# aik2mlj/polyffusion

Hardware: AMD Instinct MI355X
Metric: denoising steps/sec (8-bar prmat2c, batch 16) (higher is better)
Workload: dtype bf16x3; 1 GPU; sdf_chd8bar cond generation, batch 16 per GPU, 1000-step DDPM sampler loop body (BASELINE.json configs[1]); weights: deterministic synthetic, 41.08M params; global_batch=16, parallelism=batch-shard x1

## Files before the change

polyffusion_amd/csrc/conv_bf16x3.hip:

```cpp
#include <vector>

#include "conv_common.h"

namespace pf {

#ifdef PF_TRACE
__device__ unsigned long long g_trace[8192];
#define TR() do { if (trace_on && tslot < 2040) { g_trace[tbase + tslot++] = __builtin_amdgcn_s_memtime(); } } while (0)
#else
#define TR() do {} while (0)
#endif

typedef x3_t x3x4 __attribute__((ext_vector_type(4)));

template <int KS, int STRIDE, int TWIN, int BN>
constexpr int conv_bf3_row_pitch() {
  return (KS != 1 && STRIDE == 1 && BN >= 128) ? (TWIN * 40 + 127) / 128 * 128 : TWIN * 40;
}

#ifndef PF_KG2_RING
#define PF_KG2_RING 5
#endif
template <int KS, int BN, int KG>
constexpr bool conv_bf3_pingpong() { return KS == 3 && BN == 128 && KG == 2; }
// ... 132 lines not shown
    {
      f32x4 v = ra[i];
      if (poff[i] < 0) v = f32x4{0.f, 0.f, 0.f, 0.f};
      else if (PRO != 0) {
        if (PRO == 3) {
          v = (v - pmu[i]) * prs[i] * vsc + vsh;
        } else {
          v = v * vsc + vsh;
          if (PRO == 1) { v[0] = silu_f(v[0]); v[1] = silu_f(v[1]); v[2] = silu_f(v[2]); v[3] = silu_f(v[3]); }
        }
      }
      qh[i] = __builtin_convertvector(v, x3x4);
      const f32x4 hf = __builtin_convertvector(qh[i], f32x4);
      ql[i] = __builtin_convertvector(v - hf, x3x4);
    }
  };
  auto transformA = [&]() {
#pragma unroll
    for (int i = 0; i < NA; ++i) transformPiece(i);
  };
  auto writeA = [&](int buf) {
#pragma unroll
    for (int i = 0; i < NA; ++i) {
      const int pix = tid / KQ + i * PSTEP;
      if (pix < NPIX) {
        const int o = buf * ABUF + (pix / TWIN) * RP + (pix % TWIN) * PITCH + c4 * 4;
        *reinterpret_cast<x3x4*>(sAh + o) = qh[i];
        *reinterpret_cast<x3x4*>(sAl + o) = ql[i];
      }
    }
  };
  auto storeA = [&](int buf) { transformA(); writeA(buf); };
  auto loadW = [&](int chunk, int tap) {
    const size_t toff = ((size_t)tap * K8 + (size_t)(cbeg + chunk) * 4) * ((size_t)2 * p.Npad * 8);
#pragma unroll
    for (int j = 0; j < NW; ++j) {
      const int u = tid + j * NT;
      const int k8l = u / (2 * BN), plane = (u / BN) & 1, n = u % BN;
      rw[j] = *reinterpret_cast<const u32x4*>(static_cast<const x3_t*>(p.w) + ((size_t)(k8l * 2 + plane) * p.Npad + n0 + n) * 8 + toff);
    }
  };
  auto storeW = [&](int buf) {
    x3_t* dst = sW + buf * (TOTW * 8);
#pragma unroll
    for (int j = 0; j < NW; ++j) {
      *reinterpret_cast<u32x4*>(dst + (tid + j * NT) * 8) = rw[j];
    }
  };

  static_assert(NT % (2 * BN) == 0, "pieces of a thread must be whole k8 rows apart");
  const int wrow_b = 2 * p.Npad * 8 * 2;
  const __amdgpu_buffer_rsrc_t rsW = dma_resource(static_cast<const x3_t*>(p.w) + (size_t)n0 * 8);
  const int vw0 = (((tid / (2 * BN)) * 2 + ((tid / BN) & 1)) * p.Npad + tid % BN) * 16;
  auto gldsW = [&](int chunk, int tap, int buf) {
    const int toff = ((q * TAPS + tap) * K8 + (cbeg + chunk) * 4) * wrow_b;
#pragma unroll
    for (int j = 0; j < NW; ++j) {
      x3_t* l = sW + buf * (TOTW * 8) + (wave * 64 + j * NT) * 8;
      dma16(rsW, vw0, toff + j * (NT / (2 * BN)) * wrow_b, l);
    }
  };

  int hbase[FM];
#pragma unroll
  for (int fm = 0; fm < FM; ++fm) {
    const int pp = wm * WM + fm * 32 + (lane & 31);
    const int py = pp / TW, px = pp % TW;
    hbase[fm] = (py * STRIDE) * RP + (px * STRIDE) * PITCH + 8 * (lane >> 5);
  }
  const int wbase = ((lane >> 5) * 2 * BN + wn * WN + (lane & 31)) * 8;

  f32x16 acc[FM][FN];
#pragma unroll
  for (int fm = 0; fm < FM; ++fm)
#pragma unroll
    for (int fn = 0; fn < FN; ++fn)
#pragma unroll
      for (int r = 0; r < 16; ++r) acc[fm][fn][r] = 0.f;


  auto gnFused = [&]() {
    if constexpr (PRO == 1 || PRO == 2) {
      if (p.gn_s0) {
        gn_fused_prologue<KG * NT>(p, b, threadIdx.x, p.Hin * p.Win, reinterpret_cast<double*>(smem_all));
        const int cg = cbeg * BK;
        vsc = *reinterpret_cast<const f32x4*>(p.sc + (size_t)b * cin + cg + c4 * 4);
        vsh = *reinterpret_cast<const f32x4*>(p.sh + (size_t)b * cin + cg + c4 * 4);
        sc_ready = true;
      }
    }
  };
  if constexpr (KS == 1) {
    loadA(0); loadW(0, 0);
    gnFused();
    storeA(0); storeW(0);
    __syncthreads();
    for (int chunk = 0; chunk < nchunk; ++chunk) {
      const int nchunk1 = min(chunk + 1, nchunk - 1);
      loadW(nchunk1, 0);
      loadA(nchunk1);
      const int aoff = (chunk & 1) * ABUF;
      const x3_t* cW = sW + (chunk & 1) * (TOTW * 8) + wbase;
#pragma unroll
      for (int s = 0; s < BK / 16; ++s) {
        x3x8 ah[FM], al[FM], bh[FN], bl[FN];
#pragma unroll
        for (int fm = 0; fm < FM; ++fm) {
          ah[fm] = *reinterpret_cast<const x3x8*>(sAh + aoff + hbase[fm] + s * 16);
          al[fm] = *reinterpret_cast<const x3x8*>(sAl + aoff + hbase[fm] + s * 16);
        }
#pragma unroll
        for (int fn = 0; fn < FN; ++fn) {
          bh[fn] = *reinterpret_cast<const x3x8*>(cW + ((4 * s) * BN + fn * 32) * 8);
          bl[fn] = *reinterpret_cast<const x3x8*>(cW + ((4 * s + 1) * BN + fn * 32) * 8);
        }
#pragma unroll
        for (int fm = 0; fm < FM; ++fm)
#pragma unroll
          for (int fn = 0; fn < FN; ++fn) acc[fm][fn] = x3_mfma_32x32x16(al[fm], bh[fn], acc[fm][fn], 0, 0, 0);
#pragma unroll
        for (int fm = 0; fm < FM; ++fm)
#pragma unroll
          for (int fn = 0; fn < FN; ++fn) acc[fm][fn] = x3_mfma_32x32x16(ah[fm], bl[fn], acc[fm][fn], 0, 0, 0);
#pragma unroll
        for (int fm = 0; fm < FM; ++fm)
#pragma unroll
          for (int fn = 0; fn < FN; ++fn) acc[fm][fn] = x3_mfma_32x32x16(ah[fm], bh[fn], acc[fm][fn], 0, 0, 0);
      }
      storeW((chunk + 1) & 1);
      storeA((chunk + 1) & 1);
      __syncthreads();
    }
  } else {
    constexpr int NS = BK / 16;
    static_assert(NS == 2 && WRING >= 2 && WRING <= TAPS, "pipeline is written for two K steps per tap and a ring no deeper than a chunk's taps");
    constexpr bool DYN = TAPS % WRING != 0;
    constexpr int NAL = NA + (PRO != 0 ? 2 : 0);
    constexpr bool PP = conv_bf3_pingpong<KS, BN, KG>();
#pragma unroll
    for (int d = 0; d < (PP ? 2 : WRING); ++d) gldsW(0, d, d);
    TR();
    loadA(0);
    TR();
    gnFused();
    storeA(0);
    TR();
    asm volatile("s_waitcnt vmcnt(0) lgkmcnt(0)" ::: "memory");
    __builtin_amdgcn_s_barrier();
    x3x8 ah[FM], al[FM], bh[FN], bl[FN];
    unsigned abase[FM];
#pragma unroll
    for (int fm = 0; fm < FM; ++fm) abase[fm] = (unsigned)(size_t)(__attribute__((address_space(3))) x3_t*)(sAh + hbase[fm]);
    const unsigned wb = (unsigned)(size_t)(__attribute__((address_space(3))) x3_t*)(sW + wbase);
    constexpr int ALO = APLANE * 2;
    constexpr int WSLOT = TOTW * 16;
    static_assert(ALO + (2 * RP + 2 * PITCH) * 2 + 64 < 65536 && (DYN ? 1 : WRING) * WSLOT < 65536, "LDS immediates must fit 16 bits");
#define LD_AL1(I, AOFF, S) al[I] = lds_read128<ALO + ((AOFF) + (S) * 16) * 2>(abase[I])
#define LD_AH1(I, AOFF, S) ah[I] = lds_read128<((AOFF) + (S) * 16) * 2>(abase[I])
#define LD_BH1(I, SLOT, S) bh[I] = lds_read128<(DYN ? 0 : slot_##SLOT * WSLOT) + ((4 * (S)) * BN + (I) * 32) * 16>(DYN ? wb_##SLOT : wb)
#define LD_BL1(I, SLOT, S) bl[I] = lds_read128<(DYN ? 0 : slot_##SLOT * WSLOT) + ((4 * (S) + 1) * BN + (I) * 32) * 16>(DYN ? wb_##SLOT : wb)
#define LD_AL(AOFF, S) static_for<0, FM>([&](auto i) { LD_AL1(i.value, AOFF, S); })
#define LD_AH(AOFF, S) static_for<0, FM>([&](auto i) { LD_AH1(i.value, AOFF, S); })
#define LD_BH(SLOT, S) static_for<0, FN>([&](auto i) { LD_BH1(i.value, SLOT, S); })
#define LD_BL(SLOT, S) static_for<0, FN>([&](auto i) { LD_BL1(i.value, SLOT, S); })
#define SB() __builtin_amdgcn_sched_barrier(0)
#define FENCE() asm volatile("" ::: "memory")
    constexpr int G = FM * FN;
    auto GX = [&](auto&& f) {
      static_for<0, FM>([&](auto fm) { static_for<0, FN>([&](auto fn) {
        acc[fm.value][fn.value] = x3_mfma_32x32x16(al[fm.value], bh[fn.value], acc[fm.value][fn.value], 0, 0, 0);
// ... 593 lines not shown
```

polyffusion_amd/csrc/conv_common.h:

```cpp
#pragma once
#include <type_traits>

#include "pf_internal.h"

namespace pf {

typedef x3_t x3x8 __attribute__((ext_vector_type(8)));
typedef unsigned int u32x4 __attribute__((ext_vector_type(4)));

template <int OFF>
__device__ __forceinline__ x3x8 lds_read128(unsigned addr) {
  u32x4 v;
  constexpr int HI = OFF & ~0xFFFF, LO = OFF & 0xFFFF;
  if constexpr (HI != 0) addr += HI;
  asm volatile("ds_read_b128 %0, %1 offset:%2" : "=v"(v) : "v"(addr), "n"(LO));
  return __builtin_bit_cast(x3x8, v);
}
__device__ __forceinline__ __amdgpu_buffer_rsrc_t dma_resource(const void* base) {
  return __builtin_amdgcn_make_buffer_rsrc(const_cast<void*>(base), 0, 0x7fffffff, 0x00020000);
}
__device__ __forceinline__ void dma16(__amdgpu_buffer_rsrc_t rs, int voff, int soff, void* lds_wave_base) {
  __builtin_amdgcn_raw_ptr_buffer_load_lds(rs, (__attribute__((address_space(3))) void*)lds_wave_base, 16, voff, soff, 0, 0);
}

template <int N>
__device__ __forceinline__ void lgkm_wait() { asm volatile("s_waitcnt lgkmcnt(%0)" ::"n"(N)); }
template <int I, int N, class F>
__device__ __forceinline__ void static_for(F&& f) {
  if constexpr (I < N) { f(std::integral_constant<int, I>{}); static_for<I + 1, N>(f); }
}


struct FastDiv { unsigned mul, shr; };
static inline FastDiv make_fastdiv(int d) {
  if (d <= 1) return FastDiv{0u, 0u};
  unsigned l = 31u - (unsigned)__builtin_clz((unsigned)d);
  if (d & (d - 1)) ++l;
  const unsigned p = 31u + l;
  return FastDiv{(unsigned)(((1ull << p) + (unsigned)d - 1u) / (unsigned)d), p - 32u};
}
__device__ __forceinline__ int fdiv(int x, FastDiv f) { return f.mul ? (int)(__umulhi((unsigned)x, f.mul) >> f.shr) : x; }

struct ConvP {
  const float* x0; const float* x1; int c0, c1;
  int B, Hin, Win, Hout, Wout;
  const void* w; int N, Npad;
  const float* sc; const float* sh; const float* mean; const float* rstd;
  const float* bias; const float* sbias; int ld_sbias; const float* res; int ld_res;
  const long long* sb_rows; int sb_nrows;
  int geglu;
  float* out; int ld_out;
  float* stats;
  int tiles_x, tiles_y, nt;
  FastDiv d_tx, d_ty, d_nt, d_ks;
  int fold, fold_py, fold_px;
  const float* sx0; const float* sx1; int sc0, sc1;
  const void* sw; const float* bias2;
  void* out_planes;
  void* qkv;
  int pp;
  int ksplit; float* partial;
  const float* gn_s0; const float* gn_s1; int gn_t0, gn_t1;
  const float* gn_gamma; const float* gn_beta; float gn_eps; int gn_groups;
  int x1_bmod;
  unsigned* amax;
};

__device__ __forceinline__ void conv_shared_x1(ConvP& p, int b) {
  if (p.x1_bmod > 0) {
    const size_t d = (size_t)(b - b % p.x1_bmod);
    if (p.x1) p.x1 -= d * ((size_t)p.Hin * p.Win * p.c1);
    if (p.sx1) p.sx1 -= d * ((size_t)p.Hout * p.Wout * p.sc1);
    if (p.gn_s1) p.gn_s1 -= d * ((size_t)p.gn_t1 * p.c1 * 2);
  }
}

static inline void conv_fill_divs(ConvP& p) {
  p.d_tx = make_fastdiv(p.tiles_x); p.d_ty = make_fastdiv(p.tiles_y); p.d_nt = make_fastdiv(p.nt); p.d_ks = make_fastdiv(p.ksplit);
}

template <int NTHREADS>
__device__ __forceinline__ void gn_fused_prologue(const ConvP& p, int b, int tid_wg, int hw, double* scratch) {
  const int cin = p.c0 + p.c1, gs = cin / p.gn_groups;
  for (int c = tid_wg; c < cin; c += NTHREADS) {
    const float* s; int T, C, cl;
    if (c < p.c0) { s = p.gn_s0; T = p.gn_t0; C = p.c0; cl = c; } else { s = p.gn_s1; T = p.gn_t1; C = p.c1; cl = c - p.c0; }
    double a = 0.0, q = 0.0;
    for (int t0 = 0; t0 < T; t0 += 8) {
      float2 vv[8];
#pragma unroll
      for (int j = 0; j < 8; ++j)
        vv[j] = *reinterpret_cast<const float2*>(s + (((size_t)b * T + min(t0 + j, T - 1)) * C + cl) * 2);
#pragma unroll
      for (int j = 0; j < 8; ++j)
        if (t0 + j < T) { a += vv[j].x; q += vv[j].y; }
    }
    scratch[2 * c] = a; scratch[2 * c + 1] = q;
  }
  __syncthreads();
  float* scw = const_cast<float*>(p.sc) + (size_t)b * cin;
  float* shw = const_cast<float*>(p.sh) + (size_t)b * cin;
  for (int c = tid_wg; c < cin; c += NTHREADS) {
    const int g0 = (c / gs) * gs;
    double a = 0.0, q = 0.0;
    for (int j = 0; j < gs; ++j) { a += scratch[2 * (g0 + j)]; q += scratch[2 * (g0 + j) + 1]; }
    const double cnt = (double)gs * hw;
    const double mean = a / cnt;
    double var = q / cnt - mean * mean;
    if (var < 0.0) var = 0.0;
    const double rstd = 1.0 / sqrt(var + (double)p.gn_eps);
    const double ga = p.gn_gamma[c];
    scw[c] = (float)(rstd * ga);
    shw[c] = (float)((double)p.gn_beta[c] - mean * rstd * ga);
  }
  __threadfence_block();
  __syncthreads();
}

__device__ __forceinline__ void amax_acc(unsigned& m, float v) { m = max(m, __float_as_uint(v) & 0x7fffffffu); }
__device__ __forceinline__ void amax_acc4(unsigned& m, f32x4 v) { amax_acc(m, v[0]); amax_acc(m, v[1]); amax_acc(m, v[2]); amax_acc(m, v[3]); }
__device__ __forceinline__ void amax_flush(unsigned* slot, unsigned m) {
  if (!slot) return;
#pragma unroll
  for (int o = 32; o >= 1; o >>= 1) m = max(m, (unsigned)__shfl_xor((int)m, o));
  if ((threadIdx.x & 63) == 0 && m) atomicMax(slot, m);
}

__device__ __forceinline__ float silu_f(float v) { return v * __builtin_amdgcn_rcpf(1.0f + __expf(-v)); }
__device__ __forceinline__ float erf_as_f(float x) {
  const float ax = fabsf(x);
  const float t = __builtin_amdgcn_rcpf(fmaf(0.3275911f, ax, 1.0f));
  float pq = fmaf(1.061405429f, t, -1.453152027f);
  pq = fmaf(pq, t, 1.421413741f);
  pq = fmaf(pq, t, -0.284496736f);
  pq = fmaf(pq, t, 0.254829592f);
  const float y = 1.0f - pq * t * __expf(-ax * ax);
  return copysignf(y, x);
}
__device__ __forceinline__ float gelu_erf_f(float g) { return 0.5f * g * (1.0f + erf_as_f(g * 0.70710678118654752440f)); }

__device__ __forceinline__ void store_out(const ConvP& p, size_t idx, float v) { p.out[idx] = v; }
__device__ __forceinline__ const float* sbias_row(const ConvP& p, int b) {
  if (!p.sbias) return nullptr;
  long long r = b;
  if (p.sb_rows) { r = p.sb_rows[b]; r = r < 0 ? 0 : (r >= p.sb_nrows ? p.sb_nrows - 1 : r); }
  return p.sbias + (size_t)r * p.ld_sbias;
}
__device__ __forceinline__ size_t out_pixel(const ConvP& p, int b, int oy, int ox) {
  if (p.fold) return ((size_t)b * (2 * p.Hout) + 2 * oy + p.fold_py) * (size_t)(2 * p.Wout) + 2 * ox + p.fold_px;
  return ((size_t)b * p.Hout + oy) * p.Wout + ox;
}

__device__ __forceinline__ void quad_transpose_s1(f32x4& a, int lane) {
  const bool p1 = lane & 1;
  float s0 = p1 ? a[0] : a[1], s1 = p1 ? a[2] : a[3];
  float r0 = __builtin_bit_cast(float, __builtin_amdgcn_mov_dpp(__builtin_bit_cast(int, s0), 0xB1, 0xF, 0xF, true));
  float r1 = __builtin_bit_cast(float, __builtin_amdgcn_mov_dpp(__builtin_bit_cast(int, s1), 0xB1, 0xF, 0xF, true));
  if (p1) { a[0] = r0; a[2] = r1; } else { a[1] = r0; a[3] = r1; }
}
__device__ __forceinline__ void quad_transpose_s2(f32x4& a, int lane) {
  const bool p2 = lane & 2;
  float s0 = p2 ? a[0] : a[2], s1 = p2 ? a[1] : a[3];
  float r0 = __builtin_bit_cast(float, __builtin_amdgcn_mov_dpp(__builtin_bit_cast(int, s0), 0x4E, 0xF, 0xF, true));
  float r1 = __builtin_bit_cast(float, __builtin_amdgcn_mov_dpp(__builtin_bit_cast(int, s1), 0x4E, 0xF, 0xF, true));
  if (p2) { a[0] = r0; a[1] = r1; } else { a[2] = r0; a[3] = r1; }
}
__device__ __forceinline__ void quad_transpose(f32x4& a, int lane) { quad_transpose_s1(a, lane); quad_transpose_s2(a, lane); }
__device__ __forceinline__ float quad_sum(float v) {
  v += __builtin_bit_cast(float, __builtin_amdgcn_mov_dpp(__builtin_bit_cast(int, v), 0xB1, 0xF, 0xF, true));
  v += __builtin_bit_cast(float, __builtin_amdgcn_mov_dpp(__builtin_bit_cast(int, v), 0x4E, 0xF, 0xF, true));
  return v;
}

template <int TH, int TW, int BN, int FM, int FN, int NWM = 2>
__device__ __forceinline__ void conv_epilogue(const ConvP& p, f32x16 (&acc)[FM][FN], int b, int oy0, int ox0, int n0,
                                              int wm, int wn, int lane, int tid, float* red, bool active = true) {
  constexpr int WM = TH * TW / NWM, WN = BN / 2;
  unsigned am = 0;
  if (!active) {
    if (p.stats && !p.partial) { __syncthreads(); __syncthreads(); }
    return;
  }
  if (p.partial) {
#pragma unroll
    for (int fm = 0; fm < FM; ++fm)
#pragma unroll
      for (int r = 0; r < 16; ++r) {
        const int row = (r & 3) + 8 * (r >> 2) + 4 * (lane >> 5);
        const int pp = wm * WM + fm * 32 + row;
        const int oy = oy0 + pp / TW, ox = ox0 + pp % TW;
        if (oy >= p.Hout || ox >= p.Wout) continue;
        const size_t m = out_pixel(p, b, oy, ox);
#pragma unroll
        for (int fn = 0; fn < FN; ++fn) {
          const int n = n0 + wn * WN + fn * 32 + (lane & 31);
          if (n < p.N) p.partial[m * p.N + n] = acc[fm][fn][r];
        }
// ... 334 lines not shown
```

polyffusion_amd/csrc/conv_wino.hip:

```cpp
#include "conv_common.h"

namespace pf {

typedef x3_t x3x4 __attribute__((ext_vector_type(4)));

#ifdef PF_TRACE
__device__ unsigned long long g_wtrace[3 * 256];
#define WTR() do { if (trace_on && tslot < 255) { g_wtrace[tbase + tslot++] = __builtin_amdgcn_s_memtime(); } } while (0)
#define WTR_DECL() const bool trace_on = (threadIdx.x == 0) && (blockIdx.x == 0 || blockIdx.x == gridDim.x / 2 || blockIdx.x == gridDim.x - 1); \
                   const int tbase = blockIdx.x == 0 ? 0 : (blockIdx.x == gridDim.x - 1 ? 512 : 256); int tslot = 0; (void)tbase
#else
#define WTR() do {} while (0)
#define WTR_DECL() do {} while (0)
#endif

constexpr int WPP = 36, WRP = 18 * WPP + 8, WHALO = 18 * WRP;
constexpr int WINO_LDS = 4 * 2 * 4 * 16 * 64 * 4;

__device__ __forceinline__ void lds_barrier() {
  asm volatile("s_waitcnt lgkmcnt(0)" ::: "memory");
  __builtin_amdgcn_s_barrier();
  asm volatile("" ::: "memory");
}

template <class T>
__device__ __forceinline__ const T* uniform_ptr(const T* q) {
  const unsigned long long v = reinterpret_cast<unsigned long long>(q);
  const unsigned lo = __builtin_amdgcn_readfirstlane((unsigned)v), hi = __builtin_amdgcn_readfirstlane((unsigned)(v >> 32));
  return reinterpret_cast<const T*>(((unsigned long long)hi << 32) | lo);
}

__device__ __forceinline__ __amdgpu_buffer_rsrc_t rsrc_or_empty(const void* q) {
  return __builtin_amdgcn_make_buffer_rsrc(const_cast<void*>(q), 0, q ? 0x7fffffff : 0, 0x00020000);
}
__device__ __forceinline__ const float* sbias_row_scalar(const ConvP& p, int b) {
  if (!p.sbias) return nullptr;
  long long r = b;
  if (p.sb_rows) {
    typedef const long long __attribute__((address_space(4))) * cptr;
    r = *((cptr)(unsigned long long)(p.sb_rows + b));
    r = r < 0 ? 0 : (r >= p.sb_nrows ? p.sb_nrows - 1 : r);
  }
  return p.sbias + (size_t)r * p.ld_sbias;
}

__device__ __forceinline__ void wino_epilogue(const ConvP& p, f32x16 (&acc)[4][2][2], unsigned char* smem_all, int b, int oy0, int ox0, int n0,
                                              int ty_t, int tx_t, int wave, int lane, int tid, const float* sb, bool trace_on = false, int tbase = 0, int tslot = 0) {
  (void)trace_on; (void)tbase; (void)tslot;
  const int fh = wave >> 1, fnb = wave & 1;
  const int c8 = lane & 7, tl = lane >> 3;
  const int n = n0 + fnb * 32 + c8 * 4;
  const int pix0 = (b * p.Hout + oy0 + 8 * fh) * p.Wout + ox0 + 2 * tl;
  auto pix = [&](int u, int pp, int q) { return pix0 + (2 * u + pp) * p.Wout + q; };
  const __amdgpu_buffer_rsrc_t rsRes = rsrc_or_empty(uniform_ptr(p.res)), rsOut = rsrc_or_empty(uniform_ptr(p.out));
  f32x4 rr[4][2][2];
#pragma unroll
  for (int u = 0; u < 4; ++u)
#pragma unroll
    for (int pp = 0; pp < 2; ++pp)
#pragma unroll
      for (int q = 0; q < 2; ++q)
        rr[u][pp][q] = __builtin_bit_cast(f32x4, __builtin_amdgcn_raw_buffer_load_b128(rsRes, (pix(u, pp, q) * p.ld_res + n) * 4, 0, 0));
  const f32x4 cba = __builtin_bit_cast(f32x4, __builtin_amdgcn_raw_buffer_load_b128(rsrc_or_empty(uniform_ptr(p.bias)), n * 4, 0, 0));
  const f32x4 cbb = __builtin_bit_cast(f32x4, __builtin_amdgcn_raw_buffer_load_b128(rsrc_or_empty(uniform_ptr(sb)), n * 4, 0, 0));
  const f32x4 cbc = __builtin_bit_cast(f32x4, __builtin_amdgcn_raw_buffer_load_b128(rsrc_or_empty(uniform_ptr(p.bias2)), n * 4, 0, 0));
  lds_barrier();
  float* X = reinterpret_cast<float*>(smem_all);
#pragma unroll
  for (int h = 0; h < 2; ++h)
#pragma unroll
    for (int nb = 0; nb < 2; ++nb) {
      const int blk = h * 2 + nb;
#pragma unroll
      for (int r = 0; r < 16; ++r) {
        const float s0 = acc[0][h][nb][r] + acc[1][h][nb][r] + acc[2][h][nb][r];
        const float s1 = acc[1][h][nb][r] - acc[2][h][nb][r] - acc[3][h][nb][r];
        X[((((wave * 2 + 0) * 4 + blk) * 16 + r) * 64) + lane] = s0;
        X[((((wave * 2 + 1) * 4 + blk) * 16 + r) * 64) + lane] = s1;
      }
      __builtin_amdgcn_sched_barrier(0);
    }
  WTR();
  lds_barrier();
  WTR();
  const f32x4 cb4 = cba + cbb + cbc;
  f32x4 s1 = {0.f, 0.f, 0.f, 0.f}, s2 = s1;
  unsigned am = 0;
  const float* Xr = X + (tl & 3) * 64 + ((tl >> 2) & 1) * 32 + c8 * 4;
#pragma unroll
  for (int u = 0; u < 4; ++u)
#pragma unroll
    for (int q = 0; q < 2; ++q) {
      f32x4 sv[4];
#pragma unroll
      for (int i = 0; i < 4; ++i) sv[i] = *reinterpret_cast<const f32x4*>(Xr + ((((i * 2 + q) * 4 + wave) * 16 + 4 * u) * 64));
#pragma unroll
      for (int pp = 0; pp < 2; ++pp) {
        f32x4 v = pp == 0 ? sv[0] + sv[1] + sv[2] : sv[1] - sv[2] - sv[3];
        v = PF_X3_UNSCALE(v) + cb4 + rr[u][pp][q];
        __builtin_amdgcn_raw_buffer_store_b128(__builtin_bit_cast(u32x4, v), rsOut, (pix(u, pp, q) * p.ld_out + n) * 4, 0, 0);
        if (p.amax) amax_acc4(am, v);
        s1 += v; s2 += v * v;
      }
    }
  WTR();
  amax_flush(p.amax, am);
  if (p.stats) {
    lds_barrier();
    float* red = reinterpret_cast<float*>(smem_all);
    *reinterpret_cast<f32x4*>(red + (wave * 64 + lane) * 8) = s1;
    *reinterpret_cast<f32x4*>(red + (wave * 64 + lane) * 8 + 4) = s2;
    lds_barrier();
    if (tid < 64) {
      const int nb = tid >> 5, cc = (tid & 31) >> 2, e = tid & 3;
      float a0 = 0.f, a1 = 0.f;
#pragma unroll
      for (int h = 0; h < 2; ++h)
#pragma unroll
        for (int t8 = 0; t8 < 8; ++t8) {
          const float* q = red + ((h * 2 + nb) * 64 + t8 * 8 + cc) * 8 + e;
          a0 += q[0]; a1 += q[4];
        }
      const int tile = ty_t * p.tiles_x + tx_t;
      float* dst = p.stats + (((size_t)b * (p.tiles_x * p.tiles_y) + tile) * p.N + n0 + tid) * 2;
      dst[0] = a0; dst[1] = a1;
    }
  }
  WTR();
}

typedef float f32x2_ __attribute__((ext_vector_type(2)));
__device__ __forceinline__ f32x2_ silu2(f32x2_ v) {
  f32x2_ t = v * -1.44269504088896340736f;
  t[0] = __builtin_amdgcn_exp2f(t[0]); t[1] = __builtin_amdgcn_exp2f(t[1]);
  t = t + 1.0f;
  t[0] = __builtin_amdgcn_rcpf(t[0]); t[1] = __builtin_amdgcn_rcpf(t[1]);
  return v * t;
}

__device__ __forceinline__ f32x2_ pk_sub(f32x2_ a, f32x2_ b) { f32x2_ d; asm("v_pk_add_f32 %0, %1, %2 neg_lo:[0,1] neg_hi:[0,1]" : "=v"(d) : "v"(a), "v"(b)); return d; }
__device__ __forceinline__ f32x2_ pk_fma(f32x2_ a, f32x2_ b, f32x2_ c) { f32x2_ d; asm("v_pk_fma_f32 %0, %1, %2, %3" : "=v"(d) : "v"(a), "v"(b), "v"(c)); return d; }
__device__ __forceinline__ f32x4 sub4(f32x4 a, f32x4 b) {
  const f32x2_ l = pk_sub(f32x2_{a[0], a[1]}, f32x2_{b[0], b[1]}), h = pk_sub(f32x2_{a[2], a[3]}, f32x2_{b[2], b[3]});
  return f32x4{l[0], l[1], h[0], h[1]};
}
__device__ __forceinline__ f32x4 fma4(f32x4 a, f32x2_ s2, f32x4 c) {
  const f32x2_ l = pk_fma(f32x2_{a[0], a[1]}, s2, f32x2_{c[0], c[1]}), h = pk_fma(f32x2_{a[2], a[3]}, s2, f32x2_{c[2], c[3]});
  return f32x4{l[0], l[1], h[0], h[1]};
}

typedef x3_t x3x2 __attribute__((ext_vector_type(2)));
typedef float f32x2 __attribute__((ext_vector_type(2)));
struct SplitK { unsigned c0, c1; };
__device__ __forceinline__ SplitK split_consts() {
#ifdef PF_X3_F16
  SplitK k{0x0000BC00u, 0xBC000000u};
#else
  SplitK k{0x0000BF80u, 0xBF800000u};
#endif
  asm volatile("" : "+s"(k.c0), "+s"(k.c1));
  return k;
}
__device__ __forceinline__ float x3_sub_hi(x3x2 hp, unsigned c, float v) {
#ifdef PF_X3_F16
  return __builtin_amdgcn_fdot2(hp, __builtin_bit_cast(x3x2, c), v, false);
#else
  return __builtin_amdgcn_fdot2_f32_bf16(hp, __builtin_bit_cast(x3x2, c), v, false);
#endif
}
__device__ __forceinline__ void split4(f32x4 v, x3x4& hi, x3x4& lo, SplitK k) {
  const x3x2 h01 = __builtin_convertvector(f32x2{v[0], v[1]}, x3x2), h23 = __builtin_convertvector(f32x2{v[2], v[3]}, x3x2);
  const float l0 = x3_sub_hi(h01, k.c0, v[0]), l1 = x3_sub_hi(h01, k.c1, v[1]), l2 = x3_sub_hi(h23, k.c0, v[2]), l3 = x3_sub_hi(h23, k.c1, v[3]);
  const x3x2 q01 = __builtin_convertvector(f32x2{l0, l1}, x3x2), q23 = __builtin_convertvector(f32x2{l2, l3}, x3x2);
  hi = __builtin_shufflevector(h01, h23, 0, 1, 2, 3);
  lo = __builtin_shufflevector(q01, q23, 0, 1, 2, 3);
}

template <int DUMMY>
__global__ __launch_bounds__(256, 1) void conv_wino_pipe_kernel(ConvP p) {
  extern __shared__ __attribute__((aligned(16))) unsigned char smem_all[];
  WTR_DECL();
  WTR();
  constexpr int WIMG = WHALO + 1024;
  float* H0 = reinterpret_cast<float*>(smem_all) + 1024;
  const int tid = threadIdx.x, lane = tid & 63;
  const int wave = __builtin_amdgcn_readfirstlane(tid >> 6);

  int lid;
  {
    const int nwg = gridDim.x, orig = blockIdx.x;
    const int xcd = orig & 7, q = nwg >> 3, r = nwg & 7;
    lid = __builtin_amdgcn_readfirstlane((xcd < r ? xcd * (q + 1) : r * (q + 1) + (xcd - r) * q) + (orig >> 3));
  }
  int mt = __builtin_amdgcn_readfirstlane(fdiv(lid, p.d_nt));
  const int nti = lid - mt * p.nt;
  int t = __builtin_amdgcn_readfirstlane(fdiv(mt, p.d_tx));
  const int tx_t = mt - t * p.tiles_x; mt = t;
  const int b = __builtin_amdgcn_readfirstlane(fdiv(mt, p.d_ty));
  const int ty_t = mt - b * p.tiles_y;
  const int n0 = nti * 64, oy0 = ty_t * 16, ox0 = tx_t * 16;
  conv_shared_x1(p, b);
  const int cin = p.c0 + p.c1, nchunk = cin / 32, KK = cin / 16;
  const float* sbp = sbias_row_scalar(p, b);

  if (p.gn_s0) gn_fused_prologue<256>(p, b, tid, p.Hin * p.Win, reinterpret_cast<double*>(smem_all));

  const int sub = tid & 7;
  int* gpL = reinterpret_cast<int*>(H0 + WIMG + WHALO) + tid;
  int gpr[11];
  const int bpix = b * p.Hin * p.Win;
#pragma unroll
  for (int it = 0; it < 11; ++it) {
    const int pix = min((tid >> 3) + 32 * it, 323);
    const int row = (int)__umul24(pix, 57) >> 10, col = pix - (int)__umul24(row, 18);
    const int iy = oy0 - 1 + row, ix = ox0 - 1 + col;
    const bool inside = (unsigned)iy < (unsigned)p.Hin && (unsigned)ix < (unsigned)p.Win;
    const int gpix = inside ? (int)__umul24(iy, p.Win) + ix + 1 : 0;
    const int real4 = (int)__umul24(row, WRP / 4) + (int)__umul24(col, WPP / 4) + (sub ^ ((row >> 1) & 1));
    const int lo4 = inside ? 256 + real4 : tid;
    if (!inside) {
      *reinterpret_cast<f32x4*>(H0 + real4 * 4) = f32x4{0.f, 0.f, 0.f, 0.f};
      *reinterpret_cast<f32x4*>(H0 + WIMG + real4 * 4) = f32x4{0.f, 0.f, 0.f, 0.f};
    }
    gpr[it] = gpix | (lo4 << 20);
    gpL[it * 256] = gpr[it];
  }
  const __amdgpu_buffer_rsrc_t rsSc = dma_resource(uniform_ptr(p.sc + (size_t)b * cin)), rsSh = dma_resource(uniform_ptr(p.sh + (size_t)b * cin));
  float* scL = reinterpret_cast<float*>(gpL - tid + 11 * 256);
  float* shL = scL + cin;
  const float* px0 = uniform_ptr(p.x0);
  const float* px1 = uniform_ptr(p.x1);
  f32x4 ra[11], vsc, vsh;
  auto scRead = [&](int ct) {
    vsc = *reinterpret_cast<const f32x4*>(scL + ct * 32 + sub * 4);
    vsh = *reinterpret_cast<const f32x4*>(shL + ct * 32 + sub * 4);
  };
  int gq = 0, gst = 0;
  auto gpRead = [&](int pi) { gq = gpL[pi * 256]; };
  auto haloFetch = [&](int ct, int gpv, int skip = 0) -> f32x4 {
    const int cg = ct * 32;
    const bool first = cg < p.c0;
    const __amdgpu_buffer_rsrc_t rs = dma_resource(first ? px0 : px1);
    const int cs4 = (first ? p.c0 : p.c1) * 4, co4 = (first ? cg : cg - p.c0) * 4 + bpix * cs4;
    const int gpix = (gpv & 0xFFFFF) - 1;
    const int vo = ((int)__umul24(gpix, cs4) + sub * 16) | (gpix & (int)0x80000000u) | skip;
    return __builtin_bit_cast(f32x4, __builtin_amdgcn_raw_buffer_load_b128(rs, vo, co4, 0));
  };
  auto haloLoad = [&](int pi, int ct, int gpv, int skip = 0) { ra[pi] = haloFetch(ct, gpv, skip); };
  auto stageWhole = [&](f32x4 r, f32x4 sc4, f32x4 sh4, int gpv, float* Ht) {
    r = r * sc4 + sh4;
    const f32x2_ a = silu2(f32x2_{r[0], r[1]}), c2 = silu2(f32x2_{r[2], r[3]});
    *reinterpret_cast<f32x4*>(Ht - 1024 + (((unsigned)gpv >> 20) << 2)) = f32x4{a[0], a[1], c2[0], c2[1]};
  };
  auto scLoad = [&](int ct) {
    vsc = __builtin_bit_cast(f32x4, __builtin_amdgcn_raw_buffer_load_b128(rsSc, sub * 16, ct * 128, 0));
    vsh = __builtin_bit_cast(f32x4, __builtin_amdgcn_raw_buffer_load_b128(rsSh, sub * 16, ct * 128, 0));
  };
  auto stageA = [&](int pi) {
    gst = gpL[pi * 256];
    const f32x2_ a = silu2(f32x2_{ra[pi][0], ra[pi][1]} * f32x2_{vsc[0], vsc[1]} + f32x2_{vsh[0], vsh[1]});
    ra[pi][0] = a[0]; ra[pi][1] = a[1];
  };
  auto stageB = [&](int pi, float* Ht) {
    const f32x2_ a = silu2(f32x2_{ra[pi][2], ra[pi][3]} * f32x2_{vsc[2], vsc[3]} + f32x2_{vsh[2], vsh[3]});
    ra[pi][2] = a[0]; ra[pi][3] = a[1];
    *reinterpret_cast<f32x4*>(Ht - 1024 + (((unsigned)gst >> 20) << 2)) = ra[pi];
  };

  const int m = lane & 31, g = lane >> 5, tyl = m >> 3, txl = m & 7;
  const int ax = wave == 0 ? 0 : (wave == 2 ? 2 : 1);
  const int ay = wave == 0 ? 2 : (wave == 1 ? 2 : (wave == 2 ? 1 : 3));
  const float sigma = wave == 1 ? 1.f : -1.f;
  int ox_, oy_;
  {
    const int rx = 2 * tyl + ax, ry = 2 * tyl + ay;
    ox_ = rx * WRP + (2 * txl) * WPP + (((2 * g) ^ ((rx >> 1) & 1)) << 2);
    oy_ = ry * WRP + (2 * txl) * WPP + (((2 * g) ^ ((ry >> 1) & 1)) << 2);
    asm volatile("" : "+v"(ox_), "+v"(oy_));
  }
  const SplitK spk = split_consts();
  f32x2_ sig2 = {sigma, sigma};
  asm volatile("" : "+v"(sig2));
  f32x4 rwx[2], rwy[2], tt[4];
  x3x4 fh_[2][4][2], fl_[2][4][2];
  auto fragRead = [&](const float* Hn, int s, int h, int e, int b2) {
    int ex = ox_, ey = oy_;
    if (e) { asm volatile("v_xor_b32 %0, 4, %1" : "=v"(ex) : "v"(ox_)); asm volatile("v_xor_b32 %0, 4, %1" : "=v"(ey) : "v"(oy_)); }
#pragma unroll
    for (int bb = 0; bb < 2; ++bb) {
      rwx[bb] = *reinterpret_cast<const f32x4*>(Hn + ex + ((2 * b2 + bb) * WPP + s * 16 + h * 8 * WRP));
      rwy[bb] = *reinterpret_cast<const f32x4*>(Hn + ey + ((2 * b2 + bb) * WPP + s * 16 + h * 8 * WRP));
    }
  };
  auto fragT = [&](int b2) {
#pragma unroll
    for (int bb = 0; bb < 2; ++bb) tt[2 * b2 + bb] = fma4(rwy[bb], sig2, rwx[bb]);
  };
  auto fragV = [&](int set, int j, int e) {
    const f32x4 v = j == 0 ? sub4(tt[0], tt[2]) : (j == 1 ? tt[1] + tt[2] : (j == 2 ? sub4(tt[2], tt[1]) : sub4(tt[1], tt[3])));
    split4(v, fh_[set][j][e], fl_[set][j][e], spk);
  };

  const __amdgpu_buffer_rsrc_t rsW = dma_resource(uniform_ptr(static_cast<const x3_t*>(p.w) + ((size_t)wave * KK * p.nt + nti) * 8192));
  const int wstep = p.nt * 16384;
  x3x8 bh[4][2], bl[4][2];
  auto wLoad = [&](int j, int kk) {
#pragma unroll
    for (int nb = 0; nb < 2; ++nb) {
      bh[j][nb] = __builtin_bit_cast(x3x8, __builtin_amdgcn_raw_buffer_load_b128(rsW, lane * 16, kk * wstep + ((j * 2 + nb) * 2 + 0) * 1024, 0));
      bl[j][nb] = __builtin_bit_cast(x3x8, __builtin_amdgcn_raw_buffer_load_b128(rsW, lane * 16, kk * wstep + ((j * 2 + nb) * 2 + 1) * 1024, 0));
    }
  };

  auto wLoad1 = [&](int j, int nb, bool lo, int kk, int skip) {
    if (lo) bl[j][nb] = __builtin_bit_cast(x3x8, __builtin_amdgcn_raw_buffer_load_b128(rsW, (lane * 16) | skip, kk * wstep + ((j * 2 + nb) * 2 + 1) * 1024, 0));
    else bh[j][nb] = __builtin_bit_cast(x3x8, __builtin_amdgcn_raw_buffer_load_b128(rsW, (lane * 16) | skip, kk * wstep + ((j * 2 + nb) * 2 + 0) * 1024, 0));
  };
  f32x16 acc[4][2][2];

#define SB() __builtin_amdgcn_sched_barrier(0)
  {
    const int c1 = min(1, nchunk - 1);
#pragma unroll
    for (int pi = 0; pi < 11; ++pi) haloLoad(pi, 0, gpr[pi]);
    scLoad(0);
    const f32x4 vsc0 = vsc, vsh0 = vsh;
    f32x4 rb[3];
#pragma unroll
    for (int pi = 0; pi < 3; ++pi) rb[pi] = haloFetch(c1, gpr[pi]);
    scLoad(c1);
#pragma unroll
    for (int j = 0; j < 4; ++j) wLoad(j, 0);
    float tsc[4], tsh[4];
#pragma unroll
    for (int i = 0; i < 4; ++i) {
      const int c = min(tid + 256 * i, cin - 1);
      tsc[i] = p.sc[(size_t)b * cin + c]; tsh[i] = p.sh[(size_t)b * cin + c];
    }
    WTR();
    SB();
    {
      x3x8 z8;
#pragma unroll
      for (int e = 0; e < 8; ++e) z8[e] = (x3_t)0.f;
      asm volatile("" : "+v"(z8));
      const f32x16 z16 = {0.f, 0.f, 0.f, 0.f, 0.f, 0.f, 0.f, 0.f, 0.f, 0.f, 0.f, 0.f, 0.f, 0.f, 0.f, 0.f};
#pragma unroll
      for (int j = 0; j < 4; ++j)
#pragma unroll
        for (int h = 0; h < 2; ++h)
#pragma unroll
          for (int nb = 0; nb < 2; ++nb) {
            asm volatile("" : "+v"(z8));
            acc[j][h][nb] = x3_mfma_32x32x16(z8, z8, z16, 0, 0, 0);
          }
    }
#pragma unroll
    for (int i = 0; i < 4; ++i)
      if (tid + 256 * i < cin) { scL[tid + 256 * i] = tsc[i]; shL[tid + 256 * i] = tsh[i]; }
    SB();
#pragma unroll
    for (int pi = 0; pi < 11; ++pi) stageWhole(ra[pi], vsc0, vsh0, gpr[pi], H0);
    WTR();
#pragma unroll
    for (int pi = 0; pi < 3; ++pi) stageWhole(rb[pi], vsc, vsh, gpr[pi], H0 + WIMG);
#pragma unroll
    for (int pi = 3; pi < 9; ++pi) haloLoad(pi, c1, gpr[pi]);
    WTR();
    __syncthreads();
    WTR();
#pragma unroll
    for (int e = 0; e < 2; ++e) {
      fragRead(H0, 0, 0, e, 0); fragT(0); fragRead(H0, 0, 0, e, 1); fragT(1);
#pragma unroll
      for (int j = 0; j < 4; ++j) fragV(0, j, e);
    }
  }

  for (int chunk = 0; chunk < nchunk; ++chunk) {
    const int c1 = min(chunk + 1, nchunk - 1), c2 = min(chunk + 2, nchunk - 1);
    const int skip1 = chunk + 1 < nchunk ? 0 : (int)0x80000000u, skip2 = chunk + 2 < nchunk ? 0 : (int)0x80000000u;
    float* Hcur = H0 + (chunk & 1) * WIMG;
    float* Hnxt = H0 + ((chunk + 1) & 1) * WIMG;
    static_for<0, 4>([&](auto qc) {
      constexpr int QS = decltype(qc)::value, s = QS >> 1, h = QS & 1;
      constexpr int QN = (QS + 1) & 3, sn = QN >> 1, hn = QN & 1;
      const float* Hn = QS == 3 ? Hnxt : Hcur;
      float* Ht = QS == 3 ? Hcur : Hnxt;
      constexpr int sp0 = QS == 3 ? 0 : 3 * QS + 3, spn = QS == 2 ? 2 : 3;
      constexpr int lp0 = QS == 0 ? 9 : 3 * (QS - 1), lpn = QS == 0 ? 2 : 3;
      const int lct = QS == 0 ? c1 : c2;
      WTR();
      if constexpr (QS == 3) {
        asm volatile("s_waitcnt lgkmcnt(0)" ::: "memory");
        __builtin_amdgcn_s_barrier();
        asm volatile("" ::: "memory");
      }
      SB();
      static_for<0, 24>([&](auto kc) {
        constexpr int k = decltype(kc)::value, j = k / 6, kind = (k % 6) >> 1, nb = k & 1;
        const x3x8 ah = __builtin_shufflevector(fh_[h][j][0], fh_[h][j][1], 0, 1, 2, 3, 4, 5, 6, 7);
        const x3x8 al = __builtin_shufflevector(fl_[h][j][0], fl_[h][j][1], 0, 1, 2, 3, 4, 5, 6, 7);
        if constexpr (kind == 0) acc[j][h][nb] = x3_mfma_32x32x16(al, bh[j][nb], acc[j][h][nb], 0, 0, 0);
        else if constexpr (kind == 1) acc[j][h][nb] = x3_mfma_32x32x16(ah, bl[j][nb], acc[j][h][nb], 0, 0, 0);
        else acc[j][h][nb] = x3_mfma_32x32x16(ah, bh[j][nb], acc[j][h][nb], 0, 0, 0);
        SB();
        if constexpr (k == 0 || k == 8) fragRead(Hn, sn, hn, k / 8, 0);
        if constexpr (k == 2 || k == 10) { fragT(0); fragRead(Hn, sn, hn, k / 8, 1); }
        if constexpr (k == 4 || k == 12) { fragT(1); fragV(hn, 0, k / 8); }
        if constexpr (k == 5 || k == 6 || k == 7) fragV(hn, k - 4, 0);
        if constexpr (k == 13 || k == 14 || k == 15) fragV(hn, k - 12, 1);
        if constexpr (k >= 16 && k < 16 + 2 * spn) {
          constexpr int pi = sp0 + (k - 16) / 2;
          if constexpr (((k - 16) & 1) == 0) stageA(pi); else stageB(pi, Ht);
        }
        if constexpr (k == 3 || k == 9 || k == 11) {
          constexpr int li = k == 3 ? 0 : (k == 9 ? 1 : 2);
          if constexpr (li < lpn) haloLoad(lp0 + li, lct, gq, QS == 0 ? skip1 : skip2);
        }
        if constexpr (k == 1 || k == 7 || k == 9) {
          constexpr int li = k == 1 ? 0 : (k == 7 ? 1 : 2);
          if constexpr (li < lpn) gpRead(lp0 + li);
        }
        if constexpr (k == 15) scRead(QS == 3 ? c2 : c1);
        if constexpr (h == 1 && (k % 6) >= 2) wLoad1(j, k & 1, (k % 6) < 4, s == 0 ? chunk * 2 + 1 : c1 * 2, s == 0 ? 0 : skip1);
        SB();
      });
    });
  }
#undef SB
  WTR();
#ifdef PF_TRACE
  wino_epilogue(p, acc, smem_all, b, oy0, ox0, n0, ty_t, tx_t, wave, lane, tid, sbp, trace_on, tbase, tslot);
#else
  wino_epilogue(p, acc, smem_all, b, oy0, ox0, n0, ty_t, tx_t, wave, lane, tid, sbp);
#endif
}

bool conv_wino_eligible(const pf_conv_args& a) {
  return a.wino > 0 && a.w_wino && a.precision == PF_PREC_BF16X3 && a.ks == 3 && a.stride == 1 && !a.ups && !a.ups_fold && a.prologue == 1 &&
         a.hin % 16 == 0 && a.win % 16 == 0 && a.n % 64 == 0 && a.c0 % 32 == 0 && a.c1 % 32 == 0 && !a.geglu && !a.out_planes && !a.qkv_planes &&
         a.c0 + a.c1 <= 1024 && a.hin * a.win < (1 << 20) &&
// ... 86 lines not shown
```

polyffusion_amd/csrc/small_kernels.hip:

```cpp
#include "pf_internal.h"

namespace pf {

int num_cus() {
  static std::atomic<int> cache[64];
  int dev = 0;
  if (hipGetDevice(&dev) != hipSuccess) return 256;
  int v = cache[dev & 63].load(std::memory_order_relaxed);
  if (v == 0) {
    if (hipDeviceGetAttribute(&v, hipDeviceAttributeMultiprocessorCount, dev) != hipSuccess || v <= 0) v = 256;
    cache[dev & 63].store(v, std::memory_order_relaxed);
  }
  return v;
}

__device__ __forceinline__ float silu_s(float v) { return v / (1.0f + __expf(-v)); }

__global__ __launch_bounds__(256) void conv_in_kernel(const float* __restrict__ x, const float* __restrict__ w,
                                                      const float* __restrict__ bias, float* __restrict__ out, int B, int Cin,
                                                      int Cout, int H, int W) {
  extern __shared__ float sw[];
  const int K = Cin * 9;
  for (int i = threadIdx.x; i < Cout * K; i += 256) sw[i] = w[i];
  __syncthreads();
  const int CQ = Cout / 4;
  const size_t total = (size_t)B * H * W * CQ;
  for (size_t idx = (size_t)blockIdx.x * 256 + threadIdx.x; idx < total; idx += (size_t)gridDim.x * 256) {
    const int cq = (int)(idx % CQ);
    const size_t pix = idx / CQ;
    const int xw = (int)(pix % W), yh = (int)((pix / W) % H), b = (int)(pix / ((size_t)W * H));
    float acc[4];
#pragma unroll
    for (int j = 0; j < 4; ++j) acc[j] = bias[cq * 4 + j];
    for (int ci = 0; ci < Cin; ++ci) {
      const float* xp = x + ((size_t)b * Cin + ci) * H * W;
#pragma unroll
      for (int r = 0; r < 3; ++r) {
        const int iy = yh + r - 1;
        if (iy < 0 || iy >= H) continue;
#pragma unroll
        for (int s = 0; s < 3; ++s) {
          const int ix = xw + s - 1;
          if (ix < 0 || ix >= W) continue;
          const float v = xp[(size_t)iy * W + ix];
#pragma unroll
          for (int j = 0; j < 4; ++j) acc[j] = fmaf(v, sw[(cq * 4 + j) * K + ci * 9 + r * 3 + s], acc[j]);
        }
      }
    }
    *reinterpret_cast<float4*>(out + pix * Cout + cq * 4) = make_float4(acc[0], acc[1], acc[2], acc[3]);
  }
}

template <int CIN>
__global__ __launch_bounds__(256) void conv_in_reg_kernel(const float* __restrict__ x, const float* __restrict__ w,
                                                          const float* __restrict__ bias, float* __restrict__ out, int B,
                                                          int H, int W, float* __restrict__ stats) {
  constexpr int K = CIN * 9, T = 16, TI = T + 2, COUT = 64;
  __shared__ float sx[CIN][TI][TI + 1];
  __shared__ float sred[16][16][8];
  const int tid = threadIdx.x;
  int bid = blockIdx.x;
  const int tilesx = (W + T - 1) / T, tilesy = (H + T - 1) / T;
  const int tx = bid % tilesx; bid /= tilesx;
  const int ty = bid % tilesy;
  const int b = bid / tilesy;
  for (int u = tid; u < CIN * TI * TI; u += 256) {
    const int ci = u / (TI * TI), r = (u / TI) % TI, c = u % TI;
    const int iy = ty * T + r - 1, ix = tx * T + c - 1;
    sx[ci][r][c] = (iy >= 0 && iy < H && ix >= 0 && ix < W) ? x[((size_t)b * CIN + ci) * H * W + (size_t)iy * W + ix] : 0.f;
  }
  const int cq = tid & 15, px = tid >> 4;
  float wr[4][K], bj[4];
#pragma unroll
  for (int j = 0; j < 4; ++j) {
    bj[j] = bias[cq * 4 + j];
#pragma unroll
    for (int k = 0; k < K; ++k) wr[j][k] = w[(size_t)(cq * 4 + j) * K + k];
  }
  __syncthreads();
  const int ox = tx * T + px;
  float ssum[4] = {0.f, 0.f, 0.f, 0.f}, ssq[4] = {0.f, 0.f, 0.f, 0.f};
  if (ox < W) {
#pragma unroll 4
  for (int py = 0; py < T; ++py) {
    const int oy = ty * T + py;
    if (oy >= H) break;
    float acc[4] = {bj[0], bj[1], bj[2], bj[3]};
#pragma unroll
    for (int ci = 0; ci < CIN; ++ci)
#pragma unroll
      for (int r = 0; r < 3; ++r)
#pragma unroll
        for (int s2 = 0; s2 < 3; ++s2) {
          const float v = sx[ci][py + r][px + s2];
#pragma unroll
          for (int j = 0; j < 4; ++j) acc[j] = fmaf(v, wr[j][ci * 9 + r * 3 + s2], acc[j]);
        }
    *reinterpret_cast<float4*>(out + (((size_t)b * H + oy) * W + ox) * COUT + cq * 4) = make_float4(acc[0], acc[1], acc[2], acc[3]);
#pragma unroll
    for (int j = 0; j < 4; ++j) { ssum[j] += acc[j]; ssq[j] += acc[j] * acc[j]; }
  }
  }
  if (stats) {
#pragma unroll
    for (int j = 0; j < 4; ++j) { sred[px][cq][j] = ssum[j]; sred[px][cq][4 + j] = ssq[j]; }
    __syncthreads();
    if (tid < COUT) {
      const int q = tid >> 2, j = tid & 3;
      float a = 0.f, qq = 0.f;
#pragma unroll
      for (int c = 0; c < 16; ++c) { a += sred[c][q][j]; qq += sred[c][q][4 + j]; }
      float* dst = stats + (((size_t)b * (tilesx * tilesy) + ty * tilesx + tx) * COUT + tid) * 2;
      dst[0] = a; dst[1] = qq;
    }
  }
}

int launch_conv_in_stats_tiles(int cin, int cout, int h, int w_) { return (cin <= 2 && cout == 64) ? cdiv(h, 16) * cdiv(w_, 16) : 0; }

int launch_conv_in(const float* x, const float* w, const float* bias, float* out, int batch, int cin, int cout, int h, int w_,
                   hipStream_t stream, float* stats) {
  PF_REQUIRE(!stats || launch_conv_in_stats_tiles(cin, cout, h, w_) > 0, "conv_in: statistics only from the register-weight kernel (cin <= 2, cout == 64)");
  PF_REQUIRE(cout % 4 == 0 && (size_t)cout * cin * 9 * 4 <= 64 * 1024, "conv_in: unsupported channel counts %d->%d", cin, cout);
  const size_t total = (size_t)batch * h * w_ * (cout / 4);
  if (cin <= 2 && cout == 64) {
    const int grid = batch * cdiv(h, 16) * cdiv(w_, 16);
    if (cin == 1) hipLaunchKernelGGL(conv_in_reg_kernel<1>, dim3(grid), dim3(256), 0, stream, x, w, bias, out, batch, h, w_, stats);
    else hipLaunchKernelGGL(conv_in_reg_kernel<2>, dim3(grid), dim3(256), 0, stream, x, w, bias, out, batch, h, w_, stats);
    PF_CHECK_HIP(hipGetLastError());
    return PF_OK;
  }
  const int grid = (int)min((size_t)4096, (total + 255) / 256);
  hipLaunchKernelGGL(conv_in_kernel, dim3(grid), dim3(256), (size_t)cout * cin * 9 * sizeof(float), stream, x, w, bias, out, batch,
                     cin, cout, h, w_);
  PF_CHECK_HIP(hipGetLastError());
  return PF_OK;
}

typedef float f32x2_s __attribute__((ext_vector_type(2)));
__device__ __forceinline__ float silu_fast(float v) { return v * __builtin_amdgcn_rcpf(1.0f + __expf(-v)); }

template <int COUT>
__global__ __launch_bounds__(256) void conv_out_kernel(const float* __restrict__ x, const float* __restrict__ sc,
                                                       const float* __restrict__ sh, const float* __restrict__ w,
                                                       const float* __restrict__ bias, float* __restrict__ out, int B, int Cin,
                                                       int H, int W) {
  constexpr int T = 16, TI = T + 2, CK = 16, CP = CK + 4, NPIECE = TI * TI * (CK / 4), NP = (NPIECE + 255) / 256;
  constexpr int NPAIR = COUT / 2, ODD = COUT & 1;
  __shared__ __attribute__((aligned(16))) float sx[TI * TI * CP];
  const int tid = threadIdx.x;
  const int tilesx = (W + T - 1) / T, tilesy = (H + T - 1) / T;
  int bid = blockIdx.x;
  const int tx = bid % tilesx; bid /= tilesx;
  const int ty = bid % tilesy;
  const int b = bid / tilesy;
  const int py = tid / T, px = tid % T;
  const int c4 = tid & 3;
  unsigned goff[NP];
  int soff[NP];
  float keep[NP];
  const unsigned gsafe = (unsigned)(((b * H + min(ty * T, H - 1)) * W + min(tx * T, W - 1)) * Cin) + c4 * 4;
#pragma unroll
  for (int i = 0; i < NP; ++i) {
    const int u = tid + i * 256, pix = u >> 2;
    const int iy = ty * T + pix / TI - 1, ix = tx * T + pix % TI - 1;
    const bool in = u < NPIECE && iy >= 0 && iy < H && ix >= 0 && ix < W;
// ... 632 lines not shown
```

Measured before the change: 206.7 steps/s.

## Keep fused GroupNorm scale/shift in LDS and overlap prologue with halo loads

The fused GroupNorm prologue now also writes the per-channel scale/shift into shared memory, so the conv kernels read them from LDS instead of re-reading the global copy after a block fence. In the Winograd kernel the prologue moves after the first halo and weight loads are issued, overlapping the statistics reduction with memory traffic. The stats reduction gets a dedicated LDS region, which removes a barrier, and uses 128 threads instead of 64. The stats accumulation loop reads 16 timesteps at a time, and conv_in_reg gets launch bounds of 4 and a smaller unroll for multi-channel inputs, at the cost of larger LDS use and register pressure limits.

```diff
diff --git a/polyffusion_amd/csrc/conv_bf16x3.hip b/polyffusion_amd/csrc/conv_bf16x3.hip
--- a/polyffusion_amd/csrc/conv_bf16x3.hip
+++ b/polyffusion_amd/csrc/conv_bf16x3.hip
@@ -238,10 +238,19 @@
   auto gnFused = [&]() {
     if constexpr (PRO == 1 || PRO == 2) {
       if (p.gn_s0) {
-        gn_fused_prologue<KG * NT>(p, b, threadIdx.x, p.Hin * p.Win, reinterpret_cast<double*>(smem_all));
         const int cg = cbeg * BK;
-        vsc = *reinterpret_cast<const f32x4*>(p.sc + (size_t)b * cin + cg + c4 * 4);
-        vsh = *reinterpret_cast<const f32x4*>(p.sh + (size_t)b * cin + cg + c4 * 4);
+        float* rows = reinterpret_cast<float*>(smem_all) + 4 * cin;
+        const bool rows_fit = (size_t)cin * 24 <= (size_t)2 * APLANE * sizeof(x3_t);
+        gn_fused_prologue<KG * NT>(p, b, threadIdx.x, p.Hin * p.Win, reinterpret_cast<double*>(smem_all), rows_fit ? rows : nullptr);
+        if (rows_fit) {
+          vsc = *reinterpret_cast<const f32x4*>(rows + cg + c4 * 4);
+          vsh = *reinterpret_cast<const f32x4*>(rows + cin + cg + c4 * 4);
+          __threadfence_block();
+          __syncthreads();
+        } else {
+          vsc = *reinterpret_cast<const f32x4*>(p.sc + (size_t)b * cin + cg + c4 * 4);
+          vsh = *reinterpret_cast<const f32x4*>(p.sh + (size_t)b * cin + cg + c4 * 4);
+        }
         sc_ready = true;
       }
     }
diff --git a/polyffusion_amd/csrc/conv_common.h b/polyffusion_amd/csrc/conv_common.h
--- a/polyffusion_amd/csrc/conv_common.h
+++ b/polyffusion_amd/csrc/conv_common.h
@@ -79,25 +79,40 @@
   p.d_tx = make_fastdiv(p.tiles_x); p.d_ty = make_fastdiv(p.tiles_y); p.d_nt = make_fastdiv(p.nt); p.d_ks = make_fastdiv(p.ksplit);
 }
 
+__device__ __forceinline__ void lds_barrier() {
+  asm volatile("s_waitcnt lgkmcnt(0)" ::: "memory");
+  __builtin_amdgcn_s_barrier();
+  asm volatile("" ::: "memory");
+}
+
 template <int NTHREADS>
-__device__ __forceinline__ void gn_fused_prologue(const ConvP& p, int b, int tid_wg, int hw, double* scratch) {
+__device__ __forceinline__ void gn_fused_prologue(const ConvP& p, int b, int tid_wg, int hw, double* scratch, float* res = nullptr) {
   const int cin = p.c0 + p.c1, gs = cin / p.gn_groups;
   for (int c = tid_wg; c < cin; c += NTHREADS) {
     const float* s; int T, C, cl;
     if (c < p.c0) { s = p.gn_s0; T = p.gn_t0; C = p.c0; cl = c; } else { s = p.gn_s1; T = p.gn_t1; C = p.c1; cl = c - p.c0; }
     double a = 0.0, q = 0.0;
-    for (int t0 = 0; t0 < T; t0 += 8) {
+    const float* sb_ = s + ((size_t)b * T * C + cl) * 2;
+    if (T <= 8) {
       float2 vv[8];
 #pragma unroll
+      for (int j = 0; j < 8; ++j) vv[j] = *reinterpret_cast<const float2*>(sb_ + (size_t)min(j, T - 1) * C * 2);
+#pragma unroll
       for (int j = 0; j < 8; ++j)
-        vv[j] = *reinterpret_cast<const float2*>(s + (((size_t)b * T + min(t0 + j, T - 1)) * C + cl) * 2);
-#pragma unroll
-      for (int j = 0; j < 8; ++j)
-        if (t0 + j < T) { a += vv[j].x; q += vv[j].y; }
+        if (j < T) { a += vv[j].x; q += vv[j].y; }
+    } else {
+      for (int t0 = 0; t0 < T; t0 += 16) {
+        float2 vv[16];
+#pragma unroll
+        for (int j = 0; j < 16; ++j) vv[j] = *reinterpret_cast<const float2*>(sb_ + (size_t)min(t0 + j, T - 1) * C * 2);
+#pragma unroll
+        for (int j = 0; j < 16; ++j)
+          if (t0 + j < T) { a += vv[j].x; q += vv[j].y; }
+      }
     }
     scratch[2 * c] = a; scratch[2 * c + 1] = q;
   }
-  __syncthreads();
+  if (res) lds_barrier(); else __syncthreads();
   float* scw = const_cast<float*>(p.sc) + (size_t)b * cin;
   float* shw = const_cast<float*>(p.sh) + (size_t)b * cin;
   for (int c = tid_wg; c < cin; c += NTHREADS) {
@@ -110,9 +125,12 @@
     if (var < 0.0) var = 0.0;
     const double rstd = 1.0 / sqrt(var + (double)p.gn_eps);
     const double ga = p.gn_gamma[c];
-    scw[c] = (float)(rstd * ga);
-    shw[c] = (float)((double)p.gn_beta[c] - mean * rstd * ga);
-  }
+    const float fsc = (float)(rstd * ga), fsh = (float)((double)p.gn_beta[c] - mean * rstd * ga);
+    scw[c] = fsc;
+    shw[c] = fsh;
+    if (res) { res[c] = fsc; res[cin + c] = fsh; }
+  }
+  if (res) { lds_barrier(); return; }
   __threadfence_block();
   __syncthreads();
 }
diff --git a/polyffusion_amd/csrc/conv_wino.hip b/polyffusion_amd/csrc/conv_wino.hip
--- a/polyffusion_amd/csrc/conv_wino.hip
+++ b/polyffusion_amd/csrc/conv_wino.hip
@@ -15,13 +15,11 @@
 #endif
 
 constexpr int WPP = 36, WRP = 18 * WPP + 8, WHALO = 18 * WRP;
-constexpr int WINO_LDS = 4 * 2 * 4 * 16 * 64 * 4;
-
-__device__ __forceinline__ void lds_barrier() {
-  asm volatile("s_waitcnt lgkmcnt(0)" ::: "memory");
-  __builtin_amdgcn_s_barrier();
-  asm volatile("" ::: "memory");
-}
+constexpr int WINO_XCH = 4 * 2 * 4 * 16 * 64 * 4;
+constexpr int WINO_RED = 4 * 64 * 8 * 4;
+constexpr int WINO_LDS = WINO_XCH + WINO_RED;
+constexpr int WINO_ROWS = (1024 + (WHALO + 1024) + WHALO + 11 * 256) * 4;
+static_assert(WINO_ROWS + 24 * 1024 <= WINO_LDS, "scale / shift rows + fold scratch must fit");
 
 template <class T>
 __device__ __forceinline__ const T* uniform_ptr(const T* q) {
@@ -106,24 +104,20 @@
   WTR();
   amax_flush(p.amax, am);
   if (p.stats) {
-    lds_barrier();
-    float* red = reinterpret_cast<float*>(smem_all);
+    float* red = reinterpret_cast<float*>(smem_all + WINO_XCH);
     *reinterpret_cast<f32x4*>(red + (wave * 64 + lane) * 8) = s1;
     *reinterpret_cast<f32x4*>(red + (wave * 64 + lane) * 8 + 4) = s2;
     lds_barrier();
-    if (tid < 64) {
-      const int nb = tid >> 5, cc = (tid & 31) >> 2, e = tid & 3;
-      float a0 = 0.f, a1 = 0.f;
+    if (tid < 128) {
+      const int ch = tid & 63, kind = tid >> 6;
+      const int nb = ch >> 5, cc = (ch & 31) >> 2, e = ch & 3;
+      float a0 = 0.f;
 #pragma unroll
       for (int h = 0; h < 2; ++h)
 #pragma unroll
-        for (int t8 = 0; t8 < 8; ++t8) {
-          const float* q = red + ((h * 2 + nb) * 64 + t8 * 8 + cc) * 8 + e;
-          a0 += q[0]; a1 += q[4];
-        }
+        for (int t8 = 0; t8 < 8; ++t8) a0 += red[((h * 2 + nb) * 64 + t8 * 8 + cc) * 8 + kind * 4 + e];
       const int tile = ty_t * p.tiles_x + tx_t;
-      float* dst = p.stats + (((size_t)b * (p.tiles_x * p.tiles_y) + tile) * p.N + n0 + tid) * 2;
-      dst[0] = a0; dst[1] = a1;
+      p.stats[(((size_t)b * (p.tiles_x * p.tiles_y) + tile) * p.N + n0 + ch) * 2 + kind] = a0;
     }
   }
   WTR();
@@ -203,8 +197,6 @@
   const int cin = p.c0 + p.c1, nchunk = cin / 32, KK = cin / 16;
   const float* sbp = sbias_row_scalar(p, b);
 
-  if (p.gn_s0) gn_fused_prologue<256>(p, b, tid, p.Hin * p.Win, reinterpret_cast<double*>(smem_all));
-
   const int sub = tid & 7;
   int* gpL = reinterpret_cast<int*>(H0 + WIMG + WHALO) + tid;
   int gpr[11];
@@ -321,21 +313,34 @@
 #define SB() __builtin_amdgcn_sched_barrier(0)
   {
     const int c1 = min(1, nchunk - 1);
+    const bool fold = p.gn_s0 != nullptr;
 #pragma unroll
     for (int pi = 0; pi < 11; ++pi) haloLoad(pi, 0, gpr[pi]);
-    scLoad(0);
-    const f32x4 vsc0 = vsc, vsh0 = vsh;
-    f32x4 rb[3];
-#pragma unroll
-    for (int pi = 0; pi < 3; ++pi) rb[pi] = haloFetch(c1, gpr[pi]);
-    scLoad(c1);
-#pragma unroll
-    for (int j = 0; j < 4; ++j) wLoad(j, 0);
+    f32x4 vsc0, vsh0, rb[3];
     float tsc[4], tsh[4];
-#pragma unroll
-    for (int i = 0; i < 4; ++i) {
-      const int c = min(tid + 256 * i, cin - 1);
-      tsc[i] = p.sc[(size_t)b * cin + c]; tsh[i] = p.sh[(size_t)b * cin + c];
+    if (fold) {
+#pragma unroll
+      for (int pi = 0; pi < 3; ++pi) rb[pi] = haloFetch(c1, gpr[pi]);
+#pragma unroll
+      for (int j = 0; j < 4; ++j) wLoad(j, 0);
+      SB();
+      gn_fused_prologue<256>(p, b, tid, p.Hin * p.Win, reinterpret_cast<double*>(shL + cin), scL);
+      scRead(0);
+      vsc0 = vsc; vsh0 = vsh;
+      scRead(c1);
+    } else {
+      scLoad(0);
+      vsc0 = vsc; vsh0 = vsh;
+#pragma unroll
+      for (int pi = 0; pi < 3; ++pi) rb[pi] = haloFetch(c1, gpr[pi]);
+      scLoad(c1);
+#pragma unroll
+      for (int j = 0; j < 4; ++j) wLoad(j, 0);
+#pragma unroll
+      for (int i = 0; i < 4; ++i) {
+        const int c = min(tid + 256 * i, cin - 1);
+        tsc[i] = p.sc[(size_t)b * cin + c]; tsh[i] = p.sh[(size_t)b * cin + c];
+      }
     }
     WTR();
     SB();
@@ -355,9 +360,11 @@
             acc[j][h][nb] = x3_mfma_32x32x16(z8, z8, z16, 0, 0, 0);
           }
     }
-#pragma unroll
-    for (int i = 0; i < 4; ++i)
-      if (tid + 256 * i < cin) { scL[tid + 256 * i] = tsc[i]; shL[tid + 256 * i] = tsh[i]; }
+    if (!fold) {
+#pragma unroll
+      for (int i = 0; i < 4; ++i)
+        if (tid + 256 * i < cin) { scL[tid + 256 * i] = tsc[i]; shL[tid + 256 * i] = tsh[i]; }
+    }
     SB();
 #pragma unroll
     for (int pi = 0; pi < 11; ++pi) stageWhole(ra[pi], vsc0, vsh0, gpr[pi], H0);
diff --git a/polyffusion_amd/csrc/small_kernels.hip b/polyffusion_amd/csrc/small_kernels.hip
--- a/polyffusion_amd/csrc/small_kernels.hip
+++ b/polyffusion_amd/csrc/small_kernels.hip
@@ -53,7 +53,7 @@
 }
 
 template <int CIN>
-__global__ __launch_bounds__(256) void conv_in_reg_kernel(const float* __restrict__ x, const float* __restrict__ w,
+__global__ __launch_bounds__(256, 4) void conv_in_reg_kernel(const float* __restrict__ x, const float* __restrict__ w,
                                                           const float* __restrict__ bias, float* __restrict__ out, int B,
                                                           int H, int W, float* __restrict__ stats) {
   constexpr int K = CIN * 9, T = 16, TI = T + 2, COUT = 64;
@@ -82,7 +82,7 @@
   const int ox = tx * T + px;
   float ssum[4] = {0.f, 0.f, 0.f, 0.f}, ssq[4] = {0.f, 0.f, 0.f, 0.f};
   if (ox < W) {
-#pragma unroll 4
+#pragma unroll CIN == 1 ? 4 : 2
   for (int py = 0; py < T; ++py) {
     const int oy = ty * T + py;
     if (oy >= H) break;
```

New measurement: 207.4 steps/s (median of 6 runs). No clear change (+0.3%).
